# godhj93/bayesian-torch

Hardware: AMD Instinct MI355X
Metric: MC-samples/sec (forward+KL), Bayesian-ResNet18 CIFAR batch=128 (higher is better)
Workload: dtype f32 (bf16x3 split operands, 6 product terms, f32 accumulate); 1 GPU; cfg3: Bayesian-ResNet18 via dnn_to_bnn (Conv2dReparameterization), CIFAR 3x32x32, batch=128; samples_per_launch=32, batch=128, rng=on-chip philox, parallelism=mc1, output_stage=bn+relu+residual (+ the stem max-pool) folded into the conv kernels, launch=hip graph replay

## Files before the change

### bayesian_torch_amd/csrc/bt_fused_split.h

```cpp
#pragma once
#include "bt_fused_common.h"
#include "bt_fused_fwd.h"

namespace bt {

typedef short bf16x8 __attribute__((ext_vector_type(8)));

constexpr int kSplitSteps = 5;

template <int BM, bool FLIP = false>
constexpr int split_xpo() {
  return FLIP ? 302 : 1025;
}
template <int BN, int NP, bool FLIP = false>
constexpr int split_w_bytes() { return (FLIP ? 2 : 1) * kSplitSteps * 2 * NP * BN * 16; }
template <int BM, int NP, bool FLIP = false>
constexpr int split_x_bytes() { return split_xpo<BM, FLIP>() * (NP + (FLIP ? 1 : 0)) * 16; }
constexpr int kSplitMiscBytes = kMaxTaps * 16 + 96 + 32 + 64;
template <int BN, int BM, int NP, bool FLIP = false>
constexpr int split_stage_cap() {
  constexpr int ops = 2 * (split_w_bytes<BN, NP, FLIP>() + split_x_bytes<BM, NP, FLIP>()), pass32 = (4 * BN + 32 * (BM + 4)) * 4;
  return (NP == 1 && pass32 > ops) ? pass32 : ops;
}
template <int BN, int BM, int NP, bool FLIP = false>
constexpr int split_lds_bytes() { return split_stage_cap<BN, BM, NP, FLIP>() + kSplitMiscBytes; }

__device__ __forceinline__ void split_pieces(float v, uint32_t& h, uint32_t& m, uint32_t& l) {
  h = __float_as_uint(v) & 0xFFFF0000u;
  const float r = __fsub_rn(v, __uint_as_float(h));
  m = __float_as_uint(r) & 0xFFFF0000u;
  l = __float_as_uint(__fsub_rn(r, __uint_as_float(m)));
}
__device__ __forceinline__ uint32_t pack_hi16(uint32_t hi, uint32_t lo) {
  return __builtin_amdgcn_perm(hi, lo, 0x07060302u);
}
typedef float f32x2_t __attribute__((ext_vector_type(2)));
typedef uint32_t u32x2_t __attribute__((ext_vector_type(2)));
__device__ __forceinline__ void split_pair(float a, float b, uint32_t& h, uint32_t& m, uint32_t& l) {
  const f32x2_t v = {a, b};
  const u32x2_t hb = __builtin_bit_cast(u32x2_t, v) & 0xFFFF0000u;
  const f32x2_t r = v - __builtin_bit_cast(f32x2_t, hb);
  const u32x2_t mb = __builtin_bit_cast(u32x2_t, r) & 0xFFFF0000u;
  const f32x2_t q = r - __builtin_bit_cast(f32x2_t, mb);
  const u32x2_t lb = __builtin_bit_cast(u32x2_t, q);
  h = pack_hi16(hb.y, hb.x), m = pack_hi16(mb.y, mb.x), l = pack_hi16(lb.y, lb.x);
}

__device__ __forceinline__ uint32_t rne_pair(float lo, float hi) {
  uint32_t r;
  asm("v_cvt_pk_bf16_f32 %0, %1, %2" : "=v"(r) : "v"(lo), "v"(hi));
  return r;
}

__device__ __forceinline__ int udiv_inv(int n, int d, uint32_t inv) {
  return inv ? (int)__umulhi((uint32_t)n, inv) : (d == 1 ? n : n / d);
}
__device__ __forceinline__ uint32_t inv32(int d) { return 0xFFFFFFFFu / (uint32_t)d + 1u; }
__device__ __forceinline__ int div_small(int n, int d) { return d == 1 ? n : d == 2 ? n >> 1 : n / d; }

template <int BN, int BM, int NP, int NPW, int XM, bool FLIP = false, bool INJ = false>
__global__ __launch_bounds__(256 + 64 * NPW) void fused_split_kernel(const FwdArgs a) {
  static_assert((BN == 64 && (BM == 512 || BM == 256 || BM == 128)) || (BN == 32 && BM == 128 && !FLIP), "tile shapes of this flavour");
  static_assert(!FLIP || ((BM == 256 || BM == 128) && NP == 3), "Flipout: the 64 x 256 / 64 x 128 tiles, exact split");
  static_assert(NP >= 1 && NP <= 3 && (NP != 1 || !INJ), "pieces per value; the bf16 mode draws on chip");
  constexpr int kProducers = 64 * NPW, kThreadsAll = 256 + kProducers;
  constexpr int CWM = FLIP ? 2 : 4, CWN = 4 / CWM, WTM = BM / CWM, TN = BN / CWN / 32, TM = WTM / 32;
  constexpr int NOP = FLIP ? 2 : 1;
  constexpr int PB = 16 * (NP + (FLIP ? 1 : 0));
  constexpr int W_BYTES = split_w_bytes<BN, NP, FLIP>(), W_OP = W_BYTES / NOP, X_BYTES = split_x_bytes<BM, NP, FLIP>(), XPO = split_xpo<BM, FLIP>();
  constexpr int W_STEP = 2 * NP * BN * 16, W_HALF = NP * BN * 16, W_PIECE = BN * 16;
  constexpr int STAGE_CAP = split_stage_cap<BN, BM, NP, FLIP>();
  constexpr int SROWS = ((4 * BN + NOP * BN * (BM + 4)) * 4 <= STAGE_CAP) ? BN : 32, NPASS = BN / SROWS;
  static_assert(!FLIP || NPASS == 1, "Flipout stages both accumulator sets in one pass");

  extern __shared__ __attribute__((aligned(16))) char smem_c[];
  char* const wbuf = smem_c;
  char* const xbuf = smem_c + 2 * W_BYTES;
  float* const smem = reinterpret_cast<float*>(smem_c);
  int4* const taptab = reinterpret_cast<int4*>(smem_c + STAGE_CAP);

  unsigned long long* const dbg_ = kStamps ? a.dbg : nullptr;
  const int tid = threadIdx.x, lane = tid & 63, wave = tid >> 6;
  if (dbg_ && dbg_[201] && tid == 0) {
    dbg_[256 + 4 * blockIdx.x] = __builtin_amdgcn_s_memrealtime();
    dbg_[256 + 4 * blockIdx.x + 2] = __builtin_amdgcn_s_memtime();
    dbg_[256 + 4 * blockIdx.x + 3] = (unsigned long long)__builtin_amdgcn_s_getreg((4 << 0) | (0 << 6) | (31 << 11)) |
                                     ((unsigned long long)__builtin_amdgcn_s_getreg((20 << 0) | (0 << 6) | (31 << 11)) << 32);
  }
  const bool stamp0 = dbg_ && blockIdx.x == 0 && (tid == 0 || tid == 256);
  if (stamp0 && tid == 0) dbg_[210] = __builtin_amdgcn_s_memtime();
  const bool producer = wave >= 4;
  const int ptid = producer ? tid - 256 : tid;
  const int li = lane & 31, lh = lane >> 5;
  const int wm = wave & (CWM - 1), wn = (wave & 3) / CWM;

  int L = __builtin_amdgcn_readfirstlane(xcd_remap(blockIdx.x, a.total_blocks));
  int Lq = udiv_inv(L, a.m_tiles, a.inv_m_tiles);
  const int mt = __builtin_amdgcn_readfirstlane(L - Lq * a.m_tiles);
  L = Lq, Lq = udiv_inv(L, a.S, a.inv_S);
  const int s = __builtin_amdgcn_readfirstlane(L - Lq * a.S);
  L = Lq, Lq = udiv_inv(L, a.n_tiles, a.inv_n_tiles);
  const int nt = __builtin_amdgcn_readfirstlane(L - Lq * a.n_tiles);
  const int g = __builtin_amdgcn_readfirstlane(Lq);
  const int n0 = nt * BN;
  const bool pix = a.pixel_major != 0;
  const int t_NI = a.t_NI, t_R = a.t_R, t_Wt = a.t_Wt, RW = t_R * t_Wt, Mt = t_NI * RW;
  const int trest = udiv_inv(mt, a.n_bt, a.inv_n_bt);
  const int bt = __builtin_amdgcn_readfirstlane(mt - trest * a.n_bt);
  const int rt = __builtin_amdgcn_readfirstlane(udiv_inv(trest, a.n_ct, a.inv_n_ct)), ct = __builtin_amdgcn_readfirstlane(trest - rt * a.n_ct);
  const int b0 = bt * t_NI, r0 = rt * t_R, w0 = ct * t_Wt;
  const uint32_t inv_rw = RW > 1 ? (a.inv_rw ? a.inv_rw : inv32(RW)) : 0u;
  const uint32_t inv_wt = t_Wt > 1 ? (a.inv_wt ? a.inv_wt : inv32(t_Wt)) : 0u;
  const ColDecode cols = {b0, r0, w0, RW, Mt, t_Wt, inv_rw, inv_wt, a.B, a.Ho, a.Wo};
  const uint32_t sample = a.sample0 + (uint32_t)s;
  const int T = a.T, Cig = a.Cig;

  const RngKey key_w = weight_key(a);
  uint32_t skey_in = 0, skey_out = 0;
  if constexpr (FLIP) sign_keys(a, key_w, sample, &skey_in, &skey_out);

  int nA, dymin, dymax, dxmin, dxmax;
  {
    bool act = false;
    int4 e = make_int4(0, 0, 0, 0);
    if (lane < T) {
      const int kh = udiv_inv(lane, a.KW, a.inv_kw), kw = lane - kh * a.KW;
      e = make_int4(0, kh * a.DH, kw * a.DW, lane);
      if (pix) {
        act = (unsigned)(r0 * a.SH - a.PH + e.y) < (unsigned)a.H && (unsigned)(w0 * a.SW - a.PW + e.z) < (unsigned)a.W;
      } else {
        const int lo_h = a.PH - e.y, lo_w = a.PW - e.z;
        const int hc = lo_h > 0 ? div_small(lo_h + a.SH - 1, a.SH) : 0, wc = lo_w > 0 ? div_small(lo_w + a.SW - 1, a.SW) : 0;
        act = hc < a.Ho && hc * a.SH - lo_h < a.H && wc < a.Wo && wc * a.SW - lo_w < a.W;
        if (a.row_taps) {
          act = act && (unsigned)(r0 * a.SH - a.PH + e.y) < (unsigned)a.H;
        }
      }
    }
    const unsigned long long mask = __ballot(act);
    if (act) taptab[__popcll(mask & ((1ull << lane) - 1ull))] = e;
    int dy0 = act ? e.y : (1 << 20), dy1 = act ? e.y : -1, dx0 = act ? e.z : (1 << 20), dx1 = act ? e.z : -1;
#pragma unroll
    for (int o = 32; o > 0; o >>= 1) {
      dy0 = min(dy0, __shfl_xor(dy0, o, 64)), dy1 = max(dy1, __shfl_xor(dy1, o, 64));
      dx0 = min(dx0, __shfl_xor(dx0, o, 64)), dx1 = max(dx1, __shfl_xor(dx1, o, 64));
    }
    nA = __builtin_amdgcn_readfirstlane((int)__popcll(mask));
    dymin = __builtin_amdgcn_readfirstlane(dy0), dymax = __builtin_amdgcn_readfirstlane(dy1);
    dxmin = __builtin_amdgcn_readfirstlane(dx0), dxmax = __builtin_amdgcn_readfirstlane(dx1);
  }
  if (stamp0 && tid == 0) dbg_[211] = __builtin_amdgcn_s_memtime();

  const int G8 = Cig >> 3;
  const int ps_h = (dymax == dymin) ? 1 : a.SH, gs_h = (dymax == dymin) ? a.SH : 1;
  const int ps_w = (dxmax == dxmin) ? 1 : a.SW, gs_w = (dxmax == dxmin) ? a.SW : 1;
  const int PHt = (t_R - 1) * ps_h + (dymax - dymin) + 1, PWt = (t_Wt - 1) * ps_w + (dxmax - dxmin) + 1;
  const int x_lo = w0 * a.SW - a.PW + dxmin, y_lo = r0 * a.SH - a.PH + dymin;
  const int kmin_h = y_lo < 0 ? div_small(-y_lo + gs_h - 1, gs_h) : 0, kmin_w = x_lo < 0 ? div_small(-x_lo + gs_w - 1, gs_w) : 0;
  int kmax_h = a.H - 1 - y_lo >= 0 ? div_small(a.H - 1 - y_lo, gs_h) : -1, kmax_w = a.W - 1 - x_lo >= 0 ? div_small(a.W - 1 - x_lo, gs_w) : -1;
  kmax_h = kmax_h < PHt - 1 ? kmax_h : PHt - 1, kmax_w = kmax_w < PWt - 1 ? kmax_w : PWt - 1;
  const int NYR = kmax_h >= kmin_h ? kmax_h - kmin_h + 1 : 0, NXR = kmax_w >= kmin_w ? kmax_w - kmin_w + 1 : 0;
  const int PIMG = NYR * NXR, PCH = t_NI * PIMG;
  constexpr int ZOFF = X_BYTES - PB;
  const int SPO = (nA + 1) >> 1;
  int NO;
  if (nA <= 1) {
    NO = 2 * kSplitSteps;
  } else {
    NO = SPO == 1 ? 5 : SPO == 2 ? 2 : 1;
    static_assert(kSplitSteps == 5, "the table above");
  }
  while (NO > 1 && NO * PCH > XPO - 1) --NO;
  if (nA <= 1 && NO > 1) NO &= ~1;
  if (NO > G8) NO = G8;
  const int NQ = NO * (nA > 0 ? nA : 1);
  const int NSTEP = nA <= 1 ? (NO + 1) >> 1 : NO * SPO;
  const int NS = nA ? (G8 + NO - 1) / NO : 0;
  for (int i = tid; i < 2 * W_BYTES / 16; i += kThreadsAll) reinterpret_cast<uint4*>(smem_c)[i] = make_uint4(0, 0, 0, 0);
  if (tid < 2 * (PB / 16)) reinterpret_cast<uint4*>(xbuf + (tid / (PB / 16)) * X_BYTES + X_BYTES - PB)[tid % (PB / 16)] = make_uint4(0, 0, 0, 0);

  const float* const xs = a.x + (long long)s * a.x_sample_stride;
  constexpr uint32_t kOOB = 0x80000000u;
  auto guard_off = [](bool in, uint32_t off) -> uint32_t {
    const uint32_t m = 0u - (uint32_t)in;
    return (off & m) | (0x80000000u & ~m);
  };
  const int Cig4 = Cig;
  const int pk_bytes = a.Co * T * Cig4 * 4;
  const __amdgpu_buffer_rsrc_t r_mu = __builtin_amdgcn_make_buffer_rsrc(const_cast<float*>(a.mu_pk), 0, pk_bytes, 0x00020000);
  const __amdgpu_buffer_rsrc_t r_rs = __builtin_amdgcn_make_buffer_rsrc(const_cast<float*>(a.sig_pk), 0, pk_bytes, 0x00020000);
  const __amdgpu_buffer_rsrc_t r_x = __builtin_amdgcn_make_buffer_rsrc(const_cast<float*>(xs), 0, (int)(a.x_elems * 4), 0x00020000);
  [[maybe_unused]] const __amdgpu_buffer_rsrc_t r_ep =
      __builtin_amdgcn_make_buffer_rsrc(const_cast<float*>(INJ ? a.eps_w + (long long)s * (pk_bytes >> 2) : a.mu_pk), 0, pk_bytes, 0x00020000);
  auto ldf = [](const __amdgpu_buffer_rsrc_t& r, uint32_t byte_off) { return __builtin_bit_cast(float, __builtin_amdgcn_raw_buffer_load_b32(r, (int)byte_off, 0, 0)); };
  auto ldf4 = [](const __amdgpu_buffer_rsrc_t& r, uint32_t byte_off) { return __builtin_bit_cast(float4, __builtin_amdgcn_raw_buffer_load_b128(r, (int)byte_off, 0, 0)); };
  constexpr bool SGN = FLIP && INJ;
  [[maybe_unused]] const auto r_si = [&] {
    if constexpr (SGN) {
      const int si_bytes = (int)((a.x_elems + 15) & ~15ll);
      return __builtin_amdgcn_make_buffer_rsrc(const_cast<unsigned char*>(reinterpret_cast<const unsigned char*>(a.sign_in)) + (long long)s * si_bytes, 0, si_bytes, 0x00020000);
    } else {
      return 0;
    }
  }();
  [[maybe_unused]] const auto so_s = [&] {
    if constexpr (SGN) return reinterpret_cast<const unsigned char*>(a.sign_out) + (long long)s * (((long long)a.M * a.Co + 15) & ~15ll);
    else return 0;
  }();
  [[maybe_unused]] auto so_f = [](uint32_t word, int k) -> float { return __uint_as_float(0x3F800000u | ((word << (24 - 8 * k)) & 0x80000000u)); };

  float* const bias0 = smem;
  float* const bias1 = smem + BN;
  float* const osc = smem + 2 * BN;
  float* const osh = smem + 3 * BN;
  const bool kl_block = a.do_kl && (int)blockIdx.x < a.kl_slices;
  float* const out_s = a.out + (long long)s * a.out_elems;
  const float* const res_s = a.ep_res ? a.ep_res + (long long)s * a.ep_res_stride : nullptr;
  const uint32_t out_mis = (uint32_t)((uintptr_t)out_s | (uintptr_t)res_s);
  const bool relu = a.ep_relu != 0;
  if (stamp0 && tid == 0) dbg_[212] = __builtin_amdgcn_s_memtime();

  auto readout_quads = [&](int pass, int t0) {
    constexpr int SROW = BM + 4, QROW = BM / 4, NT_ = kThreadsAll;
    static_assert(NT_ % QROW == 0, "a thread keeps its pixel quad");
    constexpr int RSTEP = NT_ / QROW, NITc = (SROWS + RSTEP - 1) / RSTEP, U = NITc < 8 ? NITc : 8;
    const float* const stage = smem + 4 * BN;
    const int m4 = t0 % QROW, row0 = t0 / QROW;
    int bq, hq, wq;
    const bool mok = cols.decode(4 * m4, bq, hq, wq);
    const int HoWo_ = a.Ho * a.Wo;
    const int co0 = pass * SROWS + row0;
    const uint32_t obase = mok ? (uint32_t)(((bq * a.Co + g * a.Cog + n0 + co0) * a.Ho + hq) * a.Wo + wq) : 0u;
    const int rows_ok = a.Cog - n0 - pass * SROWS < SROWS ? a.Cog - n0 - pass * SROWS : SROWS;
    const float* const sp = stage + row0 * SROW + 4 * m4;
#pragma unroll
    for (int k0 = 0; k0 < NITc; k0 += U) {
      uint32_t oidx[U];
      bool okq[U];
      float4 v[U], r4[U];
#pragma unroll
      for (int u = 0; u < U; ++u) {
        const int k = k0 + u, row = row0 + k * RSTEP;
        okq[u] = k < NITc && mok && row < rows_ok;
        oidx[u] = okq[u] ? obase + (uint32_t)(k * RSTEP * HoWo_) : 0u;
        const int rr = row < SROWS ? k * RSTEP : 0;
        v[u] = *reinterpret_cast<const float4*>(sp + rr * SROW);
        if constexpr (FLIP) {
          const float4 d = *reinterpret_cast<const float4*>(sp + (SROWS + rr) * SROW);
          const int co_l = okq[u] ? co0 + k * RSTEP : 0;
          const float sc = osc[co_l], sh = osh[co_l];
          if constexpr (INJ) {
            const uint32_t sw = *reinterpret_cast<const uint32_t*>(so_s + oidx[u]);
            v[u].x = __fadd_rn(__fmul_rn(__fadd_rn(v[u].x, __fmul_rn(d.x, so_f(sw, 0))), sc), sh);
            v[u].y = __fadd_rn(__fmul_rn(__fadd_rn(v[u].y, __fmul_rn(d.y, so_f(sw, 1))), sc), sh);
            v[u].z = __fadd_rn(__fmul_rn(__fadd_rn(v[u].z, __fmul_rn(d.z, so_f(sw, 2))), sc), sh);
            v[u].w = __fadd_rn(__fmul_rn(__fadd_rn(v[u].w, __fmul_rn(d.w, so_f(sw, 3))), sc), sh);
          } else {
          v[u].x = __fadd_rn(__fmul_rn(__fadd_rn(v[u].x, __fmul_rn(d.x, hash_sign(skey_out, oidx[u]))), sc), sh);
          v[u].y = __fadd_rn(__fmul_rn(__fadd_rn(v[u].y, __fmul_rn(d.y, hash_sign(skey_out, oidx[u] + 1u))), sc), sh);
          v[u].z = __fadd_rn(__fmul_rn(__fadd_rn(v[u].z, __fmul_rn(d.z, hash_sign(skey_out, oidx[u] + 2u))), sc), sh);
          v[u].w = __fadd_rn(__fmul_rn(__fadd_rn(v[u].w, __fmul_rn(d.w, hash_sign(skey_out, oidx[u] + 3u))), sc), sh);
          }
        }
      }
      if (res_s) {
#pragma unroll
        for (int u = 0; u < U; ++u) r4[u] = *reinterpret_cast<const float4*>(res_s + oidx[u]);
#pragma unroll
        for (int u = 0; u < U; ++u)
          v[u].x = __fadd_rn(v[u].x, r4[u].x), v[u].y = __fadd_rn(v[u].y, r4[u].y), v[u].z = __fadd_rn(v[u].z, r4[u].z), v[u].w = __fadd_rn(v[u].w, r4[u].w);
      }
#pragma unroll
      for (int u = 0; u < U; ++u) {
        if (relu) v[u].x = v[u].x < 0.f ? 0.f : v[u].x, v[u].y = v[u].y < 0.f ? 0.f : v[u].y, v[u].z = v[u].z < 0.f ? 0.f : v[u].z, v[u].w = v[u].w < 0.f ? 0.f : v[u].w;
        if (okq[u]) *reinterpret_cast<float4*>(out_s + oidx[u]) = v[u];
      }
    }
  };

  const bool stage_cols = !a.out_vec4 && !pix && !a.row_taps && a.Ho * a.Wo > 4;
  auto readout_cols = [&](int pass, int t0) {
    constexpr int SROW = BM + 4, NT_ = kThreadsAll;
    static_assert(NT_ % BM == 0, "a thread keeps its column");
    constexpr int RSTEP = NT_ / BM, NITc = (SROWS + RSTEP - 1) / RSTEP;
    const float* const stage = smem + 4 * BN;
    const int c = t0 % BM, row0 = t0 / BM;
    int bq, hq, wq;
    const bool mok = cols.decode(c, bq, hq, wq);
    const int HoWo_ = a.Ho * a.Wo;
    const int co0 = pass * SROWS + row0;
    const uint32_t obase = mok ? (uint32_t)(((bq * a.Co + g * a.Cog + n0 + co0) * a.Ho + hq) * a.Wo + wq) : 0u;
    const int rows_ok = a.Cog - n0 - pass * SROWS < SROWS ? a.Cog - n0 - pass * SROWS : SROWS;
    const float* const sp = stage + row0 * SROW + c;
#pragma unroll 8
    for (int k = 0; k < NITc; ++k) {
      const int row = row0 + k * RSTEP;
      const bool ok = mok && row < rows_ok;
      const uint32_t oi = ok ? obase + (uint32_t)(k * RSTEP * HoWo_) : 0u;
      const int rr = row < SROWS ? k * RSTEP : 0;
      float v = sp[rr * SROW];
      if constexpr (FLIP) {
        const float d = sp[(SROWS + rr) * SROW];
        const int co_l = ok ? co0 + k * RSTEP : 0;
        if constexpr (INJ) v = __fadd_rn(__fmul_rn(__fadd_rn(v, __fmul_rn(d, so_f((uint32_t)so_s[oi], 0))), osc[co_l]), osh[co_l]);
        else v = __fadd_rn(__fmul_rn(__fadd_rn(v, __fmul_rn(d, hash_sign(skey_out, oi))), osc[co_l]), osh[co_l]);
      }
      if (res_s && ok) v = __fadd_rn(v, res_s[oi]);
      v = (relu && v < 0.f) ? 0.f : v;
      if (ok) out_s[oi] = v;
    }
  };

  const int prio_mode = dbg_ ? (int)dbg_[200] : 0;
  if (producer) {
    if (prio_mode == 0 && (BM == 512 || FLIP)) __builtin_amdgcn_s_setprio(3);
    constexpr int UMAX = (2 * BN * 2 * kSplitSteps + kProducers - 1) / kProducers;
    const int nunits = 2 * BN * NQ;
    uint32_t e_off[UMAX];
    int l_off[UMAX];
    int u_ol[UMAX];
    bool u_live[UMAX];
    const uint32_t inv_na = nA > 1 ? inv32(nA) : 0u;
#pragma unroll
    for (int i = 0; i < UMAX; ++i) {
      const int u = ptid + kProducers * i;
      const int uu = u < nunits ? u : 0;
      int cq = uu & 1, n = (uu >> 1) & (BN - 1), q = (uu >> 1) / BN;
      if (nA == 1 && NO > 1) {
        const uint32_t inv_no = inv32(NO);
        const int t2 = uu >> 1;
        n = (int)__umulhi((uint32_t)t2, inv_no);
        q = t2 - n * NO;
      }
      const int ol = nA > 1 ? (int)__umulhi((uint32_t)q, inv_na) : q;
      const int ai = nA > 1 ? q - ol * nA : 0;
      const int tap = nA ? taptab[ai].w : 0;
      const int st_ = nA > 1 ? ol * SPO + (ai >> 1) : (ol >> 1), hf = nA > 1 ? (ai & 1) : (ol & 1);
      const int co_g = n0 + n;
      const bool rv = co_g < a.Cog;
      const uint32_t co = (uint32_t)(g * a.Cog + (rv ? co_g : 0));
      e_off[i] = rv ? (co * (uint32_t)T + (uint32_t)tap) * (uint32_t)Cig4 + (uint32_t)(8 * ol + 4 * cq) : (kOOB >> 2);
      l_off[i] = u < nunits ? st_ * W_STEP + hf * W_HALF + (n ^ ((2 * st_ + hf) & 7)) * 16 + cq * 8 : -1;
      u_ol[i] = ol;
      u_live[i] = __builtin_amdgcn_readfirstlane(__ballot(rv && u < nunits) != 0ull ? 1 : 0) != 0;
    }
    const int wave_u0 = __builtin_amdgcn_readfirstlane(ptid & ~63);
    if (stamp0) dbg_[213] = __builtin_amdgcn_s_memtime();
    float4 mu[UMAX], rs[UMAX];
    [[maybe_unused]] float4 epl[INJ ? UMAX : 1];
    auto load_w = [&](int st) {
      const int oct0 = st * NO;
#pragma unroll
      for (int i = 0; i < UMAX; ++i) {
        if (u_live[i]) {
          const bool in = l_off[i] >= 0 && oct0 + u_ol[i] < G8 && e_off[i] != (kOOB >> 2);
          const uint32_t sb = guard_off(in, 4u * (e_off[i] + (uint32_t)(8 * oct0)));
          mu[i] = ldf4(r_mu, sb), rs[i] = ldf4(r_rs, sb);
          if constexpr (INJ) epl[i] = ldf4(r_ep, sb);
        }
      }
    };
    if (NS > 0) load_w(0);
    constexpr int PIT = (XM == 3 || XM == 4) ? ((XPO - 1) / 2 + kProducers - 1) / kProducers : (XPO - 1 + kProducers - 1) / kProducers;
    constexpr int XV = XM == 3 ? 16 : XM == 4 ? 32 : 8;
    int it_off[PIT], it_lds[PIT], it_ol[PIT];
    const bool flat = XM == 3 && a.x_flat != 0;
    const int ylo_r = y_lo + kmin_h * gs_h, nyr = flat ? 1 : NYR, W4 = flat ? a.HW >> 2 : a.W >> 2;
// ... 623 lines not shown
```

Measured before the change: 18730 MC-samples/s.

## Add a specialised one-pixel-plane path for the split conv kernel

Adds a dedicated code path for convolutions whose output plane is 1x1 (HoWo==1, HW==1), where only the centre tap touches real input. It loads only that tap's weights, double-buffers a ring of several K-steps of sampled weights in shared memory, and keeps activations in registers loaded directly from global memory instead of staging an im2col tile. The goal is to skip the padded taps and tile-staging overhead on the tiny late ResNet layers. In exchange it adds a sizeable second kernel body that raises code size and register pressure, and it only applies when XM==1 and the shape checks pass.

```diff
diff --git a/bayesian_torch_amd/csrc/bt_fused_split.h b/bayesian_torch_amd/csrc/bt_fused_split.h
--- a/bayesian_torch_amd/csrc/bt_fused_split.h
+++ b/bayesian_torch_amd/csrc/bt_fused_split.h
@@ -58,11 +58,301 @@
 __device__ __forceinline__ uint32_t inv32(int d) { return 0xFFFFFFFFu / (uint32_t)d + 1u; }
 __device__ __forceinline__ int div_small(int n, int d) { return d == 1 ? n : d == 2 ? n >> 1 : n / d; }
 
+#ifndef BT_ONE_PIXEL_STEPS
+#define BT_ONE_PIXEL_STEPS 4
+#endif
+constexpr int kOnePixelSteps = BT_ONE_PIXEL_STEPS;
+
+__device__ __forceinline__ uint32_t guarded_off(bool in, uint32_t off) {
+  const uint32_t m = 0u - (uint32_t)in;
+  return (off & m) | (0x80000000u & ~m);
+}
+
+__device__ __forceinline__ bool one_pixel_tile(const FwdArgs& a, int* tap) {
+  if (a.HoWo != 1 || a.HW != 1 || a.t_R != 1 || a.t_Wt != 1 || a.m_tiles != a.n_bt || a.updil) return false;
+  const int kh = a.DH == 1 ? a.PH : a.PH / a.DH, kw = a.DW == 1 ? a.PW : a.PW / a.DW;
+  *tap = kh * a.KW + kw;
+  return kh * a.DH == a.PH && kh < a.KH && kw * a.DW == a.PW && kw < a.KW && (a.Cig >> 3) > 0;
+}
+
+template <int BN, int NP, int NPW, bool INJ>
+__device__ __forceinline__ void split_one_pixel_tile(const FwdArgs& a, const int tap) {
+  constexpr int BM = 128, KS = kOnePixelSteps, kProducers = 64 * NPW, TN = BN / 32;
+  constexpr int W_STEP = 2 * NP * BN * 16, W_HALF = NP * BN * 16, W_PIECE = BN * 16, W_RING = KS * W_STEP;
+  constexpr int XD = 4;
+  static_assert(KS % XD == 0, "whole groups per stage");
+  static_assert(2 * W_RING + 3 * BN * 4 <= split_stage_cap<BN, BM, NP>(), "two weight images + the channel constants fit the operand buffers");
+  extern __shared__ __attribute__((aligned(16))) char smem_c[];
+  float* const bias0 = reinterpret_cast<float*>(smem_c + 2 * W_RING);
+  float* const osc = bias0 + BN;
+  float* const osh = bias0 + 2 * BN;
+
+  unsigned long long* const dbg_ = kStamps ? a.dbg : nullptr;
+  const int tid = threadIdx.x, lane = tid & 63, wave = tid >> 6;
+  const bool stamp0 = dbg_ && blockIdx.x == 0 && (tid == 0 || tid == 256);
+  if (stamp0 && tid == 0) dbg_[210] = __builtin_amdgcn_s_memtime();
+  const bool producer = wave >= 4;
+  const int ptid = producer ? tid - 256 : tid;
+  const int li = lane & 31, lh = lane >> 5;
+
+  int L = __builtin_amdgcn_readfirstlane(xcd_remap(blockIdx.x, a.total_blocks));
+  int Lq = udiv_inv(L, a.m_tiles, a.inv_m_tiles);
+  const int mt = __builtin_amdgcn_readfirstlane(L - Lq * a.m_tiles);
+  L = Lq, Lq = udiv_inv(L, a.S, a.inv_S);
+  const int s = __builtin_amdgcn_readfirstlane(L - Lq * a.S);
+  L = Lq, Lq = udiv_inv(L, a.n_tiles, a.inv_n_tiles);
+  const int nt = __builtin_amdgcn_readfirstlane(L - Lq * a.n_tiles);
+  const int g = __builtin_amdgcn_readfirstlane(Lq);
+  const int n0 = nt * BN, b0 = mt * a.t_NI;
+  const uint32_t sample = a.sample0 + (uint32_t)s;
+  const int T = a.T, Cig = a.Cig, G8 = Cig >> 3;
+  const RngKey key_w = weight_key(a);
+
+  const int NO = G8 < 2 * KS ? (G8 + 7) & ~7 : 2 * KS;
+  const int NSTEPS = (G8 + 1) >> 1, NS = (NSTEPS + KS - 1) / KS;
+
+  const float* const xs = a.x + (long long)s * a.x_sample_stride;
+  constexpr uint32_t kOOB = 0x80000000u;
+  const int pk_bytes = a.Co * T * Cig * 4;
+  const __amdgpu_buffer_rsrc_t r_mu = __builtin_amdgcn_make_buffer_rsrc(const_cast<float*>(a.mu_pk), 0, pk_bytes, 0x00020000);
+  const __amdgpu_buffer_rsrc_t r_rs = __builtin_amdgcn_make_buffer_rsrc(const_cast<float*>(a.sig_pk), 0, pk_bytes, 0x00020000);
+  const __amdgpu_buffer_rsrc_t r_x = __builtin_amdgcn_make_buffer_rsrc(const_cast<float*>(xs), 0, (int)(a.x_elems * 4), 0x00020000);
+  [[maybe_unused]] const __amdgpu_buffer_rsrc_t r_ep =
+      __builtin_amdgcn_make_buffer_rsrc(const_cast<float*>(INJ ? a.eps_w + (long long)s * (pk_bytes >> 2) : a.mu_pk), 0, pk_bytes, 0x00020000);
+  auto ldf4 = [](const __amdgpu_buffer_rsrc_t& r, uint32_t byte_off) { return __builtin_bit_cast(float4, __builtin_amdgcn_raw_buffer_load_b128(r, (int)byte_off, 0, 0)); };
+  const bool kl_block = a.do_kl && (int)blockIdx.x < a.kl_slices;
+  if (stamp0 && tid == 0) dbg_[211] = dbg_[212] = __builtin_amdgcn_s_memtime();
+
+  if (producer) {
+    constexpr int UMAX = (2 * BN * 2 * KS + kProducers - 1) / kProducers;
+    const int nunits = 2 * BN * NO;
+    const uint32_t inv_no = inv32(NO);
+    uint32_t e_off[UMAX];
+    int l_off[UMAX];
+    int u_ol[UMAX];
+    bool u_live[UMAX];
+#pragma unroll
+    for (int i = 0; i < UMAX; ++i) {
+      const int u = ptid + kProducers * i;
+      const int uu = u < nunits ? u : 0;
+      const int cq = uu & 1, t2 = uu >> 1;
+      const int n = (int)__umulhi((uint32_t)t2, inv_no), ol = t2 - n * NO;
+      const int co_g = n0 + n;
+      const bool rv = co_g < a.Cog;
+      const uint32_t co = (uint32_t)(g * a.Cog + (rv ? co_g : 0));
+      e_off[i] = rv ? (co * (uint32_t)T + (uint32_t)tap) * (uint32_t)Cig + (uint32_t)(8 * ol + 4 * cq) : (kOOB >> 2);
+      l_off[i] = u < nunits ? (ol >> 1) * W_STEP + (ol & 1) * W_HALF + (n ^ (ol & 7)) * 16 + cq * 8 : -1;
+      u_ol[i] = ol;
+      u_live[i] = __builtin_amdgcn_readfirstlane(__ballot(rv && u < nunits) != 0ull ? 1 : 0) != 0;
+    }
+    if (stamp0) dbg_[213] = dbg_[214] = __builtin_amdgcn_s_memtime();
+    float4 mu[UMAX], rs[UMAX];
+    [[maybe_unused]] float4 epl[INJ ? UMAX : 1];
+    auto load_w = [&](int st) {
+      const int oct0 = st * NO;
+#pragma unroll
+      for (int i = 0; i < UMAX; ++i) {
+        if (u_live[i]) {
+          const bool in = l_off[i] >= 0 && oct0 + u_ol[i] < G8 && e_off[i] != (kOOB >> 2);
+          const uint32_t sb = guarded_off(in, 4u * (e_off[i] + (uint32_t)(8 * oct0)));
+          mu[i] = ldf4(r_mu, sb), rs[i] = ldf4(r_rs, sb);
+          if constexpr (INJ) epl[i] = ldf4(r_ep, sb);
+        }
+      }
+    };
+    load_w(0);
+    if (stamp0) dbg_[215] = __builtin_amdgcn_s_memtime();
+    const bool pstamp = dbg_ && blockIdx.x == 0 && tid == 256;
+    for (int st = 0; st < NS; ++st) {
+      if (pstamp && st < 60) dbg_[128 + 2 * st] = __builtin_amdgcn_s_memtime();
+      char* const Wt = smem_c + (st & 1) * W_RING;
+      const int oct0 = st * NO;
+      float ep[UMAX][4];
+#pragma unroll
+      for (int i = 0; i < UMAX; ++i)
+        if (u_live[i]) {
+          if constexpr (INJ) ep[i][0] = epl[i].x, ep[i][1] = epl[i].y, ep[i][2] = epl[i].z, ep[i][3] = epl[i].w;
+          else philox_normal4(key_w, sample, (e_off[i] + (uint32_t)(8 * oct0)) >> 2, ep[i]);
+        }
+#pragma unroll
+      for (int i = 0; i < UMAX; ++i) {
+        if (u_live[i]) {
+          const float m4[4] = {mu[i].x, mu[i].y, mu[i].z, mu[i].w}, s4[4] = {rs[i].x, rs[i].y, rs[i].z, rs[i].w};
+          if constexpr (NP == 1) {
+            float w4[4];
+#pragma unroll
+            for (int j = 0; j < 4; ++j) w4[j] = __fadd_rn(m4[j], __fmul_rn(s4[j], ep[i][j]));
+            if (l_off[i] >= 0) *reinterpret_cast<uint2*>(Wt + l_off[i]) = make_uint2(rne_pair(w4[0], w4[1]), rne_pair(w4[2], w4[3]));
+          } else {
+            uint32_t wh[4], wm_[4], wl[4];
+#pragma unroll
+            for (int j = 0; j < 4; ++j)
+              split_pieces(__fadd_rn(m4[j], __fmul_rn(s4[j], ep[i][j])), wh[j], wm_[j], wl[j]);
+            if (l_off[i] >= 0) {
+              char* const dst = Wt + l_off[i];
+              *reinterpret_cast<uint2*>(dst) = make_uint2(pack_hi16(wh[1], wh[0]), pack_hi16(wh[3], wh[2]));
+              if constexpr (NP >= 2) *reinterpret_cast<uint2*>(dst + W_PIECE) = make_uint2(pack_hi16(wm_[1], wm_[0]), pack_hi16(wm_[3], wm_[2]));
+              if constexpr (NP == 3) *reinterpret_cast<uint2*>(dst + 2 * W_PIECE) = make_uint2(pack_hi16(wl[1], wl[0]), pack_hi16(wl[3], wl[2]));
+            }
+          }
+        } else if (l_off[i] >= 0) {
+          char* const dst = Wt + l_off[i];
+#pragma unroll
+          for (int p = 0; p < NP; ++p) *reinterpret_cast<uint2*>(dst + p * W_PIECE) = make_uint2(0u, 0u);
+        }
+      }
+      if (st + 1 < NS) load_w(st + 1);
+      if (pstamp && st < 60) dbg_[128 + 2 * st + 1] = __builtin_amdgcn_s_memtime();
+      __syncthreads();
+    }
+    if (ptid < BN) {
+      const ChannelConsts c = channel_consts<false, INJ>(a, key_w, s, g, n0 + ptid);
+      bias0[ptid] = c.bias0, osc[ptid] = c.scale, osh[ptid] = c.shift;
+    }
+    __syncthreads();
+  } else {
+    const int wm = wave;
+    KlSlice<1024> kls;
+    if (kl_block) kls.open(a, ptid);
+    const int col = wm * 32 + li, b = b0 + col;
+    const bool xok = col < a.t_NI && b < a.B;
+    const uint32_t xb = (uint32_t)(4 * (b * a.Ci + g * Cig));
+    float xr[XD][8];
+    auto load_x = [&](float (&d)[8], int step) {
+      const int o = 2 * step + lh;
+      const bool in = xok && o < G8;
+      const float4 v0 = ldf4(r_x, guarded_off(in, xb + (uint32_t)(32 * o))), v1 = ldf4(r_x, guarded_off(in, xb + (uint32_t)(32 * o + 16)));
+      d[0] = v0.x, d[1] = v0.y, d[2] = v0.z, d[3] = v0.w, d[4] = v1.x, d[5] = v1.y, d[6] = v1.z, d[7] = v1.w;
+    };
+#pragma unroll
+    for (int q = 0; q < XD; ++q) {
+      load_x(xr[q], q);
+      __builtin_amdgcn_sched_barrier(0);
+    }
+    int wlq[4];
+#pragma unroll
+    for (int q = 0; q < 4; ++q) wlq[q] = lh * W_HALF + (li ^ ((2 * q + lh) & 7)) * 16;
+
+    f32x16 acc[TN];
+#pragma unroll
+    for (int i = 0; i < TN; ++i)
+#pragma unroll
+      for (int r = 0; r < 16; ++r) acc[i][r] = 0.f;
+
+    const bool cstamp = dbg_ && blockIdx.x == 0 && tid == 0;
+    if (cstamp) dbg_[216] = dbg_[0] = __builtin_amdgcn_s_memtime();
+    for (int st = 0; st < NS; ++st) {
+      __syncthreads();
+      if (cstamp && st < 60) dbg_[2 + 2 * st] = __builtin_amdgcn_s_memtime();
+      const char* const Wt = smem_c + (st & 1) * W_RING;
+      const int step0 = st * KS;
+      const int nstep = NSTEPS - step0 < KS ? NSTEPS - step0 : KS;
+      for (int q4 = 0; q4 < nstep; q4 += 4) {
+        const char* const wq = Wt + q4 * W_STEP;
+#pragma unroll
+        for (int u = 0; u < 4; ++u) {
+          bf16x8 wf[TN][NP];
+#pragma unroll
+          for (int i = 0; i < TN; ++i)
+#pragma unroll
+            for (int p = 0; p < NP; ++p) wf[i][p] = *reinterpret_cast<const bf16x8*>(wq + wlq[u] + u * W_STEP + p * W_PIECE + i * 32 * 16);
+          const float(&v)[8] = xr[u];
+          bf16x8 xf[NP];
+          if constexpr (NP == 1) {
+            xf[0] = __builtin_bit_cast(bf16x8, make_uint4(rne_pair(v[0], v[1]), rne_pair(v[2], v[3]), rne_pair(v[4], v[5]), rne_pair(v[6], v[7])));
+          } else {
+            uint32_t ph[8], pm[8], pl[8];
+#pragma unroll
+            for (int c = 0; c < 8; ++c) split_pieces(v[c], ph[c], pm[c], pl[c]);
+            xf[0] = __builtin_bit_cast(bf16x8, make_uint4(pack_hi16(ph[1], ph[0]), pack_hi16(ph[3], ph[2]), pack_hi16(ph[5], ph[4]), pack_hi16(ph[7], ph[6])));
+            xf[1] = __builtin_bit_cast(bf16x8, make_uint4(pack_hi16(pm[1], pm[0]), pack_hi16(pm[3], pm[2]), pack_hi16(pm[5], pm[4]), pack_hi16(pm[7], pm[6])));
+            if constexpr (NP == 3)
+              xf[2] = __builtin_bit_cast(bf16x8, make_uint4(pack_hi16(pl[1], pl[0]), pack_hi16(pl[3], pl[2]), pack_hi16(pl[5], pl[4]), pack_hi16(pl[7], pl[6])));
+          }
+          load_x(xr[u], step0 + q4 + u + 4);
+#pragma unroll
+          for (int i = 0; i < TN; ++i) {
+            acc[i] = __builtin_amdgcn_mfma_f32_32x32x16_bf16(xf[0], wf[i][0], acc[i], 0, 0, 0);
+            if constexpr (NP >= 2) {
+              acc[i] = __builtin_amdgcn_mfma_f32_32x32x16_bf16(xf[0], wf[i][1], acc[i], 0, 0, 0);
+              acc[i] = __builtin_amdgcn_mfma_f32_32x32x16_bf16(xf[1], wf[i][0], acc[i], 0, 0, 0);
+            }
+            if constexpr (NP == 3) {
+              acc[i] = __builtin_amdgcn_mfma_f32_32x32x16_bf16(xf[0], wf[i][2], acc[i], 0, 0, 0);
+              acc[i] = __builtin_amdgcn_mfma_f32_32x32x16_bf16(xf[1], wf[i][1], acc[i], 0, 0, 0);
+              acc[i] = __builtin_amdgcn_mfma_f32_32x32x16_bf16(xf[2], wf[i][0], acc[i], 0, 0, 0);
+            }
+          }
+          __builtin_amdgcn_sched_barrier(0);
+        }
+      }
+      if (cstamp && st < 60) dbg_[2 + 2 * st + 1] = __builtin_amdgcn_s_memtime();
+      if (kl_block) kls.group(a);
+    }
+    if (cstamp) dbg_[1] = __builtin_amdgcn_s_memtime();
+
+    float* const out_s = a.out + (long long)s * a.out_elems;
+    const float* const res_s = a.ep_res ? a.ep_res + (long long)s * a.ep_res_stride : nullptr;
+    const bool relu = a.ep_relu != 0;
+    const int c_lim = (a.t_NI < a.B - b0 ? a.t_NI : a.B - b0) - wm * 32 - 4 * lh;
+    const uint32_t oi0 = (uint32_t)((b0 + wm * 32 + 4 * lh) * a.Co + g * a.Cog + n0 + li);
+    bool cok[TN];
+#pragma unroll
+    for (int i = 0; i < TN; ++i) cok[i] = n0 + i * 32 + li < a.Cog;
+    float rr[16][TN];
+#pragma unroll
+    for (int r = 0; r < 16; ++r) {
+      const int row = (r & 3) + 8 * (r >> 2);
+#pragma unroll
+      for (int i = 0; i < TN; ++i) {
+        rr[r][i] = 0.f;
+        if (res_s && row < c_lim && cok[i]) rr[r][i] = res_s[oi0 + (uint32_t)(row * a.Co + i * 32)];
+      }
+    }
+    if (kl_block) {
+      const double wsum = kls.rest(a);
+      if (lane == 0) __hip_atomic_store(&a.slots[(int)blockIdx.x * 4 + wave], wsum, __ATOMIC_RELAXED, __HIP_MEMORY_SCOPE_AGENT);
+      asm volatile("s_waitcnt vmcnt(0)" ::: "memory");
+    }
+    __syncthreads();
+    if (kl_block && wave == 0) {
+      int last = 0;
+      if (lane == 0) last = (__hip_atomic_fetch_add(a.counter, 1u, __ATOMIC_RELAXED, __HIP_MEMORY_SCOPE_AGENT) == (unsigned)a.kl_slices - 1u) ? 1 : 0;
+      if (__builtin_amdgcn_readfirstlane(last)) kl_close(a, kl_slot_sum(a, 4 * a.kl_slices, lane), lane);
+    }
+    if (cstamp) dbg_[120] = dbg_[121] = dbg_[122] = __builtin_amdgcn_s_memtime();
+    float bsv[TN], scv[TN], shv[TN];
+#pragma unroll
+    for (int i = 0; i < TN; ++i) bsv[i] = bias0[i * 32 + li], scv[i] = osc[i * 32 + li], shv[i] = osh[i * 32 + li];
+#pragma unroll
+    for (int r = 0; r < 16; ++r) {
+#pragma unroll
+      for (int i = 0; i < TN; ++i) {
+        if ((r & 3) + 8 * (r >> 2) < c_lim && cok[i]) {
+          float v = __fadd_rn(__fmul_rn(__fadd_rn(acc[i][r], bsv[i]), scv[i]), shv[i]);
+          if (res_s) v = __fadd_rn(v, rr[r][i]);
+          v = (relu && v < 0.f) ? 0.f : v;
+          out_s[oi0 + (uint32_t)(((r & 3) + 8 * (r >> 2)) * a.Co + i * 32)] = v;
+        }
+      }
+    }
+    if (cstamp) dbg_[123] = dbg_[126] = __builtin_amdgcn_s_memtime();
+  }
+}
+
 template <int BN, int BM, int NP, int NPW, int XM, bool FLIP = false, bool INJ = false>
 __global__ __launch_bounds__(256 + 64 * NPW) void fused_split_kernel(const FwdArgs a) {
   static_assert((BN == 64 && (BM == 512 || BM == 256 || BM == 128)) || (BN == 32 && BM == 128 && !FLIP), "tile shapes of this flavour");
   static_assert(!FLIP || ((BM == 256 || BM == 128) && NP == 3), "Flipout: the 64 x 256 / 64 x 128 tiles, exact split");
   static_assert(NP >= 1 && NP <= 3 && (NP != 1 || !INJ), "pieces per value; the bf16 mode draws on chip");
+  if constexpr (XM == 1 && !FLIP) {
+    static_assert(BM == 128 && NPW == 8, "the tile of the 1x1 planes");
+    int tap1;
+    if (one_pixel_tile(a, &tap1)) {
+      split_one_pixel_tile<BN, NP, NPW, INJ>(a, tap1);
+      return;
+    }
+  }
   constexpr int kProducers = 64 * NPW, kThreadsAll = 256 + kProducers;
   constexpr int CWM = FLIP ? 2 : 4, CWN = 4 / CWM, WTM = BM / CWM, TN = BN / CWN / 32, TM = WTM / 32;
   constexpr int NOP = FLIP ? 2 : 1;
```

Measured after the change: 19130 MC-samples/s (median of 6 runs). 1.02x the previous value.
